# fabriziosestito/policy-server

Hardware: AMD Instinct MI355X
Metric: admission requests evaluated/sec (node) at 64 policies; HBM GB/s vs peak (higher is better)
Workload: dtype u8; 1 GPU; C4: 1000000 synthetic Pod AdmissionReviews per GPU x 64 compiled policies (c4_64.yml: 22 psp-capabilities, 21 psp-apparmor, 21 safe-labels); config=c4_64, total_requests=1000000, policies=64, parallelism=dp1 (request shards)

## Files before the change

### include/kwgpu.h

```cpp
#ifndef KWGPU_H
#define KWGPU_H

#include <stddef.h>
#include <stdint.h>

#ifdef __cplusplus
extern "C" {
#endif

enum {
  KW_OK = 0,
  KW_E_INVALID_ID = 1,
  KW_E_INIT = 2,
  KW_E_NOT_FOUND = 3,
  KW_E_BOOTSTRAP = 4,
  KW_E_ENGINE = 5,
  KW_E_GROUP_REHYDRATE = 6,
  KW_E_ARG = 16,
  KW_E_PAYLOAD = 17,
  KW_E_DEVICE = 18,
  KW_E_NOSPACE = 19
};

enum { KW_MODE_PROTECT = 0, KW_MODE_MONITOR = 1 };
// ... 117 lines not shown
int kw_batch_to_device(kw_batch *b, int device);
int kw_batch_to_device_async(kw_batch *b, int device, void *stream);
int kw_stream_create(int device, void **stream);
void kw_stream_destroy(void *stream);
void kw_batch_destroy(kw_batch *b);

int kw_debug_host_walk(const kw_env *env, const kw_batch *b, const int32_t *policies, uint32_t npol,
                       int origin, uint32_t *out);

int kw_debug_plan(const kw_env *env, kw_batch *b, const int32_t *policies, uint32_t npol, int origin, uint32_t *out,
                  int cap);

int kw_debug_copy_jobs(const kw_env *env, kw_batch *b, const int32_t *policies, uint32_t npol, int origin,
                       uint32_t *out, size_t cap, size_t *needed);

int kw_debug_reorder(const kw_batch *b, uint64_t *perm, size_t cap, uint64_t *split, kw_batch **out);

int kw_validate_batch(const kw_env *env, kw_batch *b, const int32_t *policies, uint32_t npol,
                      int origin, void *stream);
int kw_validate_rows(const kw_env *env, kw_batch *b, const int32_t *row_policy, int origin,
                     void *stream);
int kw_batch_verdicts(kw_batch *b, uint32_t *host_out, size_t count);
int kw_validate_host(const kw_env *env, kw_batch *b, const int32_t *policies, uint32_t npol, int origin,
                     int device, uint32_t *out, size_t count, uint32_t chunk_rows);
int kw_batch_pin_host(kw_batch *b, int device);
int kw_host_alloc(int device, size_t bytes, void **out);
void kw_host_free(void *p);
int kw_batch_wide_arg(const kw_batch *b, uint64_t row, int32_t policy, uint64_t *value);
int kw_batch_group_causes(const kw_batch *b, uint64_t row, int32_t policy, uint32_t verdict, uint64_t *words,
                          size_t nwords, size_t *needed);
// ... 41 lines not shown
```

### policy-server_amd/csrc/bulk.cpp

```cpp
#include <algorithm>
#include <chrono>
#include <cstdio>
#include <cstring>
#include <optional>

#include "bulkplan.hpp"
#include "knobs.hpp"
#include "pass.hpp"
#include "plan.hpp"
#include "upload.hpp"

namespace kw {
namespace {

using clk = std::chrono::steady_clock;
double since(clk::time_point a) { return std::chrono::duration<double, std::milli>(clk::now() - a).count(); }

struct BulkTimes {
  double layout = 0, plan = 0, prep = 0, desc = 0, fill = 0, enq = 0, out = 0, first = -1, wait = 0;
};

constexpr uint64_t kRing = 4;

struct Res {
// ... 228 lines not shown
        HIPCHK(hipMemcpyAsync(dslot, hslot, pk, hipMemcpyHostToDevice, s_in));
        HIPCHK(launch_scatter(sa, s_in));
      }
    } else {
      for (const CopySeg& c : segs)
        HIPCHK(hipMemcpyAsync(D.cols + ((uint8_t*)c.dst - st), c.dst, c.bytes, hipMemcpyHostToDevice, s_in));
    }
    t.enq += since(t1);
    return KW_OK;
  }

  int stage_descs(uint64_t k) {
    const auto td = clk::now();
    cd.clear();
    co.assign(1, 0u);
    if (int rc = build_descs(kb->b, pl.geom, 0, kb->b.n, tb[k], tb[k + 1], 128, &cd, &co)) return rc;
    co[0] = (uint32_t)(co.size() - 1);
    if (cd.size() > dcap) {
      HIPCHK(hipStreamSynchronize(res->s_in.s));
      HIPCHK(hipStreamSynchronize(sc));
      dcap = cd.size() + cd.size() / 4 + 64;
      if (int rc = alloc_descs()) return rc;
    } else if (k >= 2) {
      HIPCHK(hipEventSynchronize(res->ev[3 * (k - 2)]));
    }
    if (!cd.empty()) memcpy((TileDesc*)res->hdesc.p + (k & 1) * dcap, cd.data(), cd.size() * sizeof(TileDesc));
    t.desc += since(td);
    return KW_OK;
  }

  int launch(uint64_t k) {
// ... 115 lines not shown
```

### policy-server_amd/csrc/capi.cpp

```cpp
#include <hip/hip_runtime.h>

#include <algorithm>
#include <cstdio>
#include <cstdlib>
#include <cstring>
#include <memory>
#include <string>
#include <thread>
#include <vector>

#include "../../include/kwgpu.h"
#include "automaton.hpp"
#include "batch.hpp"
#include "devbatch.hpp"
#include "env.hpp"
#include "kernels.hpp"
#include "knobs.hpp"
#include "metrics.hpp"
#include "pass.hpp"
#include "plan.hpp"
#include "service.hpp"
#include "slotplan.hpp"
#include "upload.hpp"
#include "yaml.hpp"
// ... 539 lines not shown
  kb->dev = host_view(kb);
  const DeviceBatch& D = *kb->dev;
  const Batch& B = dev_rows(kb);
  PassPlan plan;
  int rc = plan_pass(env, kb, policies, npol, nullptr, origin, false, &plan);
  std::vector<uint32_t> w;
  if (rc == KW_OK) {
    const void* cols[kMaxCopyJobs] = {D.req_flags, D.ctr_off, D.lbl_off, D.ctr_flags, D.capadd_off, D.capdrop_off};
    for (int m = 0; m < (int)NSTR; ++m) cols[6 + 2 * m] = D.str[m].off, cols[7 + 2 * m] = D.str[m].bytes;
    w.push_back((uint32_t)plan.regions.size());
    for (const PassPlan::Region& rg : plan.regions) {
      const TileArgs& T = rg.geom;
      std::vector<TileDesc> desc;
      std::vector<uint32_t> ovf;
      const uint64_t ntiles = (rg.hi - rg.lo + T.rows - 1) / T.rows;
      if ((rc = build_descs(B, T, rg.lo, rg.hi, 0, ntiles, 4096, &desc, &ovf))) break;
      for (uint32_t v : {T.rows, T.njobs, (uint32_t)desc.size(), (uint32_t)ovf.size(), (uint32_t)rg.lo, (uint32_t)rg.hi, T.lds_bytes,
                         (uint32_t)D.split})
        w.push_back(v);
      for (uint32_t v : {T.o_rf, T.o_coff, T.o_loff, T.o_cflags, T.o_cadd, T.o_cdrop}) w.push_back(v);
      w.insert(w.end(), T.o_so, T.o_so + NSTR);
      w.insert(w.end(), T.o_sb, T.o_sb + NSTR);
      for (uint32_t j = 0; j < T.njobs; ++j) {
        const CopyJob& q = T.jobs[j];
        uint32_t col = 0xffffffffu;
        for (uint32_t c = 0; c < kMaxCopyJobs; ++c)
          if ((c < 6 || T.o_sb[(c - 6) / 2]) && q.base == (uint64_t)(uintptr_t)cols[c] && col == 0xffffffffu) col = c;
        for (uint32_t v : {col, copy_lds(q.code), (q.code & kCjX4) ? 16u : 4u, q.code}) w.push_back(v);
      }
      for (const TileDesc& d : desc) {
        const uint32_t* dw = (const uint32_t*)&d;
// ... 4 lines not shown
          for (uint32_t v : {(uint32_t)sp.byte_off, (uint32_t)(sp.byte_off >> 32), sp.count}) w.push_back(v);
        }
      }
      w.insert(w.end(), ovf.begin(), ovf.end());
    }
  }
  kb->dev->verdicts = nullptr;
  kb->dev = std::move(saved);
  if (rc) return rc;
  *needed = w.size();
  if (cap < w.size()) return KW_E_NOSPACE;
  std::copy(w.begin(), w.end(), out);
  return KW_OK;
}

int kw_debug_reorder(const kw_batch* kb, uint64_t* perm, size_t cap, uint64_t* split, kw_batch** out) {
  if (!kb || !split || !out || (!perm && kb->b.n) || cap < kb->b.n) return KW_E_ARG;
  std::vector<uint64_t> p;
  *split = split_rows(kb->b, &p);
  if (!*split) {
    p.resize(kb->b.n);
    for (uint64_t r = 0; r < kb->b.n; ++r) p[r] = r;
  }
  auto nb = std::make_unique<kw_batch>();
  RowOrder o;
  permute_batch(kb->b, p, &nb->b, true, &o);
  std::copy(p.begin(), p.end(), perm);
  *out = nb.release();
  return KW_OK;
}
// ... 136 lines not shown
```

### policy-server_amd/csrc/kernels.hip

```cpp
#include <hip/hip_runtime.h>

#include <algorithm>
#include <array>
#include <cstddef>
#include <mutex>

#include "../../include/kwgpu.h"
#include "imgscan.hpp"
#include "kernels.hpp"


namespace kw {

typedef uint32_t u32x4 __attribute__((ext_vector_type(4)));

__device__ inline uint32_t lit_word(const uint32_t* base, uint32_t i, uint32_t sh, uint32_t len) {
  const uint32_t w = align_bytes(base[i + 1], base[i], sh);
  const uint32_t rem = len - 4u * i;
  return rem >= 4u ? w : (w & ((1u << (8u * rem)) - 1u));
}

template <bool BATCH, int N = 8>
__device__ inline uint32_t lit_lookup(const uint8_t* rec, const uint8_t* bytes, uint32_t b, uint32_t e) {
  const DevLit* L = (const DevLit*)rec;
// ... 1123 lines not shown
      if (ck + 1 < t.nchunk) {
        if (DYNB && tid == 0) l_nx[3] = 0;
        lds_barrier();
        mark(4);
      }
    }
    const uint64_t p3_end = timing ? clock64() : 0;
    lds_barrier();
    if (timing) sg_add(SG_P3_WAIT, clock64() - p3_end);
    mark(4);
    tile = next;
    next = dyn ? dbase + l_nx[cur] : next + wpx;
  }
  if (timing && tid == 0) {
    ph[6] = clock64() - t_begin;
    for (int k = 0; k < 8; ++k) a.phase[(uint64_t)blockIdx.x * kPhaseWords + (uint32_t)k] = ph[k];
  }
  if (dyn && tid == 0) {
    uint32_t* done = a.sched + 256u + xcd * 32u;
    __threadfence();
    if (atomicAdd(done, 1u) == wpx - 1u) {
      atomicExch(cnt, 0u);
      atomicExch(done, 0u);
    }
  }
  (void)lane;
  (void)wave;
}

constexpr int kOverflowThreads = 256;
// ... 410 lines not shown
```

### policy-server_amd/csrc/kernels.hpp

```cpp
#pragma once
#include <hip/hip_runtime.h>

#include <cstdint>

#include "kwdev.hpp"
#include "slots.hpp"

namespace kw {

enum Str : uint32_t { S_NS = 0, S_IMG, S_AA, S_CAPADD, S_CAPDROP, S_LK, S_LV, NSTR };

struct WideRec {
  uint32_t row_lo, row_hi, policy, value;
};

struct EvalArgs {
  const uint8_t* blob;
  uint64_t nrows;
  uint64_t ndesc;
  uint32_t npol;
  int32_t origin;
  const uint8_t* req_flags;
  const uint32_t* ctr_off;
  const uint32_t* lbl_off;
// ... 5 lines not shown
  uint16_t *g_ns, *g_aa, *g_img, *g_capadd, *g_capdrop, *g_lk, *g_lv;
  const uint16_t *nfa_lv, *nfa_img;
  uint32_t* wide_count;
  WideRec* wide_rec;
  uint32_t wide_cap;
  uint64_t* wide_groups;
  uint32_t nwide;
  const uint32_t* rowcol;
  uint64_t* phase;
};
enum Seg : uint32_t {
  SG_P1_LABEL = 0, SG_P1_CAPSTR, SG_P1_CTR, SG_P1_IMAGE, SG_P1_REQ, SG_P2_CTR, SG_P2_LABEL, SG_P2_REQ,
  SG_P1_BUSY, SG_P1_WAIT, SG_P2_BUSY, SG_P2_WAIT, SG_P0_WAIT, SG_P3_BUSY, SG_P3_WAIT,
  SG_START,
  SG_P0_TOP, SG_P0_REQ, SG_P0_STR,
  kSegWords = 19
};
constexpr uint32_t kPhaseWords = 8 + kSegWords;

constexpr uint32_t kSlotRows = 64;
#ifndef KW_THREADS
#define KW_THREADS 256
#endif
constexpr uint32_t kSlotThreads = KW_THREADS;
constexpr uint32_t kLdsGranule = 1280, kLdsGranules = 128;
constexpr uint32_t lds_workgroups_per_cu(uint32_t bytes) {
  const uint32_t g = (bytes + kLdsGranule - 1) / kLdsGranule;
  return g ? kLdsGranules / g : kLdsGranules;
}
constexpr uint32_t kFeatImg = 1, kFeatLbl = 2, kFeatCtr = 4, kFeatGrp = 8, kFeatAll = 15;
constexpr uint32_t kFeatNfa = 16;
constexpr uint32_t kFeatRng = 32;
#ifndef KW_PREFETCH
// ... 75 lines not shown
  uint32_t debug;
  uint32_t lds_bytes;
};

struct alignas(16) TileDesc {
  uint32_t cb, ce, lb, le, kab, kae, kdb, kde;
  uint32_t sa[NSTR];
  uint32_t pad0;
  uint32_t nv[NSTR];
  uint32_t fits;
  uint32_t r0lo, r0hi, nr;
  uint32_t pad[4];
};
static_assert(sizeof(TileDesc) == 128, "TileDesc layout");

void build_copy_jobs(TileArgs* T, const void* const cols[6]);

hipError_t launch_evaluate_tiles(const EvalArgs& a, const TileArgs& t, const TileArgs* d_t, const TileDesc* d_desc,
                                 uint32_t grid, hipStream_t s);
struct WideGroupArgs {
  uint32_t prog_off, prog_len;
  uint32_t col;
  uint32_t nmem, midx_off;
  uint32_t okw, rejb;
  uint32_t cause_off, cause_words;
  uint32_t errw;
  uint32_t kind;
  uint32_t mutw;
};

// ... 64 lines not shown
```

### policy-server_amd/csrc/knobs.hpp

```cpp
#pragma once
#include <climits>
#include <cstddef>
#include <cstdint>

namespace kw {

enum Knob : int {
  KW_STREAM_POOL, KW_HOST_THREADS, KW_L2_PREFETCH, KW_KV_GLOBAL, KW_NO_MPACK,
  KW_BULK_DEBUG, KW_BULK_SAMPLE, KW_BULK_PACK, KW_BULK_CHUNK, KW_BULK_RAMP, KW_BULK_DIRECT, KW_BULK_DEPTH,
  KW_SCHED, KW_SPLIT, KW_GROUP_FORM, KW_POISON_VERDICTS, KW_FLATTEN_THREADS,
  KW_SLOT_ROWS, KW_HEAVY_ROWS, KW_HEAVY_CTR, KW_GLOBAL_TABLES, KW_TILE_SPLIT, KW_ROUND_SPLIT,
  KW_TILE_QUANTILE, KW_TILE_DEBUG,
  KW_NKNOBS
};

enum class KnobKind : uint8_t {
  On,
  Off,
  Present,
  Int,
  Double,
  Str
};

struct KnobRow {
  const char* name;
  KnobKind kind;
// ... 31 lines not shown
    knob_flag("KW_BULK_DIRECT", KnobKind::On, kLatched, kNoPlan, "bulk path: read back straight into pinned output"),
    knob_int("KW_BULK_DEPTH", kLatched, kNoPlan, -1, 0, INT_MAX, kClamp, "bulk path: chunks in flight (0: unbounded; unset: 2 or 3)"),
    knob_flag("KW_SCHED", KnobKind::Str, kLive, kPlans, "static / dynamic: force one tile schedule"),
    knob_int("KW_SPLIT", kLive, kPlans, -1, INT_MIN, INT_MAX, kClamp, "0: never split light / heavy rows, 1: whenever both exist"),
    knob_flag("KW_GROUP_FORM", KnobKind::Str, kLive, kPlans, "script: compile every group expression as a script"),
    knob_flag("KW_POISON_VERDICTS", KnobKind::Off, kLive, kPlans, "fill the verdict words with a sentinel before a pass"),
    knob_int("KW_FLATTEN_THREADS", kLive, kNoPlan, 0, 1, INT_MAX, kClamp, "JSON flatten threads (unset: the hardware's, at most 16)"),
    knob_int("KW_SLOT_ROWS", kLive, kPlans, 0, 8, 255, kElseUnset, "force the tile height"),
    knob_int("KW_HEAVY_ROWS", kLive, kPlans, 0, 8, 255, kElseUnset, "force the heavy region's tile height"),
    knob_int("KW_HEAVY_CTR", kLive, kPlans, 5, 1, INT_MAX, kElseUnset, "containers above which a request is heavy"),
    knob_flag("KW_GLOBAL_TABLES", KnobKind::Off, kLive, kPlans, "classifier tables read from global memory"),
    knob_real("KW_TILE_SPLIT", kPlans, 0.02, "share of tiles a capacity choice may split"),
    knob_real("KW_ROUND_SPLIT", kPlans, 0.02, "share of a taller tile's tiles that may need a second P1 round"),
    knob_real("KW_TILE_QUANTILE", kPlans, 0.0, "force the capacity quantile (unset: chosen per batch)"),
    knob_int("KW_TILE_DEBUG", kLive, kPlans, 0, INT_MIN, INT_MAX, kClamp, "kernel phase ablation bits; 256: print the plan"),
};

constexpr bool knob_name_is(const char* a, const char* b) {
  while (*a && *a == *b) ++a, ++b;
  return *a == *b;
}
#define KW_KNOB_ROW(K) static_assert(knob_name_is(kKnobs[K].name, #K), "kKnobs is not in Knob order")
KW_KNOB_ROW(KW_STREAM_POOL); KW_KNOB_ROW(KW_HOST_THREADS); KW_KNOB_ROW(KW_L2_PREFETCH); KW_KNOB_ROW(KW_KV_GLOBAL);
KW_KNOB_ROW(KW_NO_MPACK); KW_KNOB_ROW(KW_BULK_DEBUG); KW_KNOB_ROW(KW_BULK_SAMPLE); KW_KNOB_ROW(KW_BULK_PACK);
KW_KNOB_ROW(KW_BULK_CHUNK); KW_KNOB_ROW(KW_BULK_RAMP); KW_KNOB_ROW(KW_BULK_DIRECT); KW_KNOB_ROW(KW_BULK_DEPTH);
KW_KNOB_ROW(KW_SCHED); KW_KNOB_ROW(KW_SPLIT); KW_KNOB_ROW(KW_GROUP_FORM); KW_KNOB_ROW(KW_POISON_VERDICTS);
KW_KNOB_ROW(KW_FLATTEN_THREADS); KW_KNOB_ROW(KW_SLOT_ROWS); KW_KNOB_ROW(KW_HEAVY_ROWS); KW_KNOB_ROW(KW_HEAVY_CTR);
KW_KNOB_ROW(KW_GLOBAL_TABLES); KW_KNOB_ROW(KW_TILE_SPLIT); KW_KNOB_ROW(KW_ROUND_SPLIT); KW_KNOB_ROW(KW_TILE_QUANTILE);
KW_KNOB_ROW(KW_TILE_DEBUG);
#undef KW_KNOB_ROW

uint64_t kw_knob_hash();

namespace knob_detail {

const char* env(const KnobRow& r);
bool parse_bool(const KnobRow& r);
int parse_int(const KnobRow& r);
double parse_double(const KnobRow& r);

template <Knob K>
bool latched_bool() {
  static const bool v = parse_bool(kKnobs[K]);
  return v;
// ... 57 lines not shown
```

### policy-server_amd/csrc/pass.cpp

```cpp
#include "pass.hpp"

#include <atomic>
#include <chrono>
#include <cstdio>
#include <cstring>
#include <memory>

#include "knobs.hpp"
#include "plan.hpp"

namespace kw {

int upload_env(kw_env* env, int device) {
  if (device < 0) return KW_OK;
  HIPCHK(hipSetDevice(device));
  HIPCHK(hipMalloc(&env->e.d_blob, env->e.blob.size()));
  HIPCHK(hipMemcpy(env->e.d_blob, env->e.blob.data(), env->e.blob.size(), hipMemcpyHostToDevice));
  env->e.device = device;
  return KW_OK;
}

int build_descs(const Batch& B, const TileArgs& T, uint64_t lo, uint64_t hi, uint64_t t0, uint64_t t1, uint64_t range,
                std::vector<TileDesc>* desc, std::vector<uint32_t>* ovf) {
  auto make = [&](uint64_t r0, uint64_t r1, TileDesc* dp) {
    TileDesc& d = *dp;
    memset(&d, 0, sizeof(d));
    d.r0lo = (uint32_t)r0;
    d.r0hi = (uint32_t)(r0 >> 32);
    d.nr = (uint32_t)(r1 - r0);
    d.cb = B.ctr_off[r0];
    d.ce = B.ctr_off[r1];
    d.lb = B.lbl_off[r0];
    d.le = B.lbl_off[r1];
    d.kab = B.capadd_off[d.cb];
    d.kae = B.capadd_off[d.ce];
    d.kdb = B.capdrop_off[d.cb];
    d.kde = B.capdrop_off[d.ce];
    bool fits = d.ce - d.cb <= T.cmax && d.kae - d.kab <= T.kmax && d.kde - d.kdb <= T.kmax && d.le - d.lb <= T.lmax;
    for (int m = 0; m < (int)NSTR; ++m) {
      if (!T.o_sb[m]) continue;
      uint64_t g0, g1;
      str_range(B, m, r0, r1, &g0, &g1);
      const StrCol& c = host_str(B, m);
      d.sa[m] = c.off[g0] & ~15u;
      d.nv[m] = (((c.off[g1] + 15u) & ~15u) - d.sa[m]) / 16u;
      fits = fits && d.nv[m] * 16u <= T.sb_cap[m];
    }
    d.fits = fits ? 1u : 0u;
    return fits;
  };
  const size_t nq = (size_t)((t1 - t0 + range - 1) / range);
  std::vector<std::vector<TileDesc>> qdesc(nq);
  std::vector<std::vector<uint32_t>> qovf(nq);
  std::atomic<bool> too_far{false};
  HostWorkers::get().run(nq, [&](size_t q) {
    std::vector<std::pair<uint64_t, uint64_t>> todo;
    std::vector<TileDesc>& dv = qdesc[q];
    dv.reserve((size_t)range + range / 64);
    for (uint64_t tile = t0 + q * range, te = std::min<uint64_t>(t1, t0 + (q + 1) * range); tile < te; ++tile) {
      todo.assign(1, {lo + tile * T.rows, std::min<uint64_t>(hi, lo + (tile + 1) * T.rows)});
      while (!todo.empty()) {
        const auto [r0, r1] = todo.back();
        todo.pop_back();
        TileDesc d;
        if (make(r0, r1, &d)) {
          dv.push_back(d);
        } else if (r1 - r0 > 1) {
          const uint64_t mid = r0 + (r1 - r0) / 2;
          todo.push_back({mid, r1});
          todo.push_back({r0, mid});
        } else {
          if (r0 > 0xffffffffull) too_far = true;
          qovf[q].push_back((uint32_t)r0);
        }
      }
    }
  });
  if (too_far) return KW_E_ARG;
  for (size_t q = 0; q < nq; ++q) {
    desc->insert(desc->end(), qdesc[q].begin(), qdesc[q].end());
    ovf->insert(ovf->end(), qovf[q].begin(), qovf[q].end());
  }
  return KW_OK;
}

static int upload_tile_descs(const Batch& B, DeviceBatch* D, const PassPlan& plan, hipStream_t s) {
  uint64_t key = 1469598103934665603ull;
  auto mix = [&](uint64_t v) { key = (key ^ v) * 1099511628211ull; };
  for (const PassPlan::Region& rg : plan.regions) {
    const TileArgs& T = rg.geom;
    mix(rg.lo);
    mix(rg.hi);
    mix(T.rows);
    mix(T.cmax);
    mix(T.kmax);
    mix(T.lmax);
    for (int m = 0; m < (int)NSTR; ++m) {
      mix(T.o_sb[m] != 0);
      mix(T.sb_cap[m]);
    }
  }
  if (D->desc && D->desc_valid && key == D->desc_key) return KW_OK;
  const bool dbg = Knobs::on<KW_BULK_DEBUG>();
  const auto t0 = std::chrono::steady_clock::now();
  std::vector<TileDesc> desc;
  std::vector<uint32_t> ovf{0};
  if (plan.regions.size() > 2) return KW_E_ARG;
  uint64_t at[2] = {0, 0}, nd[2] = {0, 0};
  for (size_t k = 0; k < plan.regions.size(); ++k) {
    const PassPlan::Region& rg = plan.regions[k];
    const uint64_t ntiles = (rg.hi - rg.lo + rg.geom.rows - 1) / rg.geom.rows;
    at[k] = desc.size();
    desc.reserve(desc.size() + ntiles + ntiles / 64 + 1);
    if (int rc = build_descs(B, rg.geom, rg.lo, rg.hi, 0, ntiles, 4096, &desc, &ovf)) return rc;
    nd[k] = desc.size() - at[k];
  }
  ovf[0] = (uint32_t)(ovf.size() - 1);
  const auto t1 = std::chrono::steady_clock::now();
  HIPCHK(hipStreamSynchronize(s));
  D->h_desc = std::move(desc);
  D->h_ovf = std::move(ovf);
  if (int rc = ensure(&D->desc, &D->desc_cap, std::max<size_t>(D->h_desc.size(), 1))) return rc;
  if (int rc = ensure(&D->overflow, &D->overflow_cap, D->h_ovf.size())) return rc;
  if (!D->h_desc.empty())
    HIPCHK(hipMemcpyAsync(D->desc, D->h_desc.data(), D->h_desc.size() * sizeof(TileDesc), hipMemcpyHostToDevice, s));
  D->ndesc = D->h_desc.size();
  for (int k = 0; k < 2; ++k) {
    D->reg_desc[k] = at[k];
    D->reg_ndesc[k] = nd[k];
  }
  HIPCHK(hipMemcpyAsync(D->overflow, D->h_ovf.data(), D->h_ovf.size() * sizeof(uint32_t), hipMemcpyHostToDevice, s));
  D->n_overflow = D->h_ovf[0];
// ... 164 lines not shown
          g[SG_P1_CTR] / wt, g[SG_P1_IMAGE] / wt, g[SG_P1_REQ] / wt, g[SG_P2_BUSY] / wt, g[SG_P2_WAIT] / wt,
          g[SG_P2_CTR] / wt, g[SG_P2_LABEL] / wt, g[SG_P2_REQ] / wt, g[SG_P3_BUSY] / wt, g[SG_P3_WAIT] / wt,
          g[SG_P0_TOP] / wt, g[SG_P0_REQ] / wt, g[SG_P0_STR] / wt);
  const uint32_t nx = std::min(8u, grid);
  uint32_t late = 0;
  double spread = 0;
  for (uint32_t x = 0; x < nx; ++x) {
    std::vector<uint64_t> st;
    for (uint32_t q = x; q < grid; q += nx) st.push_back(ph[(size_t)q * kPhaseWords + 8 + SG_START]);
    std::sort(st.begin(), st.end());
    for (uint64_t v : st) late += v > st[0] + 2000;
    spread = std::max(spread, (double)(st.back() - st[0]) / 100.0);
  }
  fprintf(stderr, "[kw start] launch %zu: %u of %u workgroups started > 20 us after their XCD's first (widest spread %.1f us)\n",
          launch, late, grid, spread);
}

static int run_pass(kw_batch* kb, PassPlan& plan, bool timed, hipStream_t s) {
  DeviceBatch& D = *kb->dev;
  EvalArgs A;
  if (int rc = prepare_pass(kb, plan, s, &A)) return rc;
  const bool phases = (plan.geom.debug & 512u) != 0;
  void* d_phase = nullptr;
  uint32_t gmax = 0;
  for (const PassPlan::Region& rg : plan.regions) gmax = std::max(gmax, rg.grid);
  const size_t phase_bytes = (size_t)gmax * kPhaseWords * sizeof(uint64_t);
  if (phases) {
    HIPCHK(hipMalloc(&d_phase, phase_bytes));
    A.phase = (uint64_t*)d_phase;
  }
// ... 264 lines not shown
```

### policy-server_amd/csrc/pass.hpp

```cpp
#pragma once
#include <hip/hip_runtime.h>

#include <algorithm>
#include <cstdint>
#include <vector>

#include "devbatch.hpp"

#define HIPCHK(x)                             \
  do {                                        \
    hipError_t _e = (x);                      \
    if (_e != hipSuccess) return KW_E_DEVICE; \
  } while (0)

namespace kw {

template <typename T>
int ensure(T** p, size_t* cap, size_t n) {
  if (*cap >= n && *p) return KW_OK;
  int dev = 0;
  HIPCHK(hipGetDevice(&dev));
  dev_pool().release(dev, *p, *cap * sizeof(T));
  *p = nullptr;
  const size_t want = BlockPool::cls(std::max<size_t>(n, 1) * sizeof(T)) / sizeof(T);
  void* q = nullptr;
  HIPCHK(dev_pool().alloc(dev, want * sizeof(T), &q));
  *p = (T*)q;
  *cap = want;
  return KW_OK;
}

int upload_env(kw_env* env, int device);

int build_descs(const Batch& B, const TileArgs& T, uint64_t lo, uint64_t hi, uint64_t t0, uint64_t t1, uint64_t range,
                std::vector<TileDesc>* desc, std::vector<uint32_t>* ovf);

int ensure_overflow_classes(const Batch& B, DeviceBatch* D, const TileArgs& T, EvalArgs* A);

int prepare_pass(kw_batch* kb, PassPlan& plan, hipStream_t s, EvalArgs* out_args, bool descs = true);

int run_validate(const kw_env* env, kw_batch* kb, PassPlan& plan, int origin, bool timed, hipStream_t s);

int validate_common(const kw_env* env, kw_batch* kb, const int32_t* policies, uint32_t npol, const int32_t* row_policy,
                    int origin, PassPlan* plan);

int validate_cached(const kw_env* env, kw_batch* kb, const int32_t* policies, uint32_t npol, int origin, PassPlan** out);

int validate_timed(const kw_env* env, kw_batch* b, const int32_t* policies, uint32_t npol, int origin, int warmup, int reps,
                   kw_timing* out);

// ... 6 lines not shown
```

### policy-server_amd/kwgpu/__init__.py

```python
import ctypes as C
import json

from . import _native as N
from ._native import KwSoa, KwTiming

PROTECT, MONITOR = N.KW_MODE_PROTECT, N.KW_MODE_MONITOR
VALIDATE, AUDIT = N.KW_ORIGIN_VALIDATE, N.KW_ORIGIN_AUDIT


class RequestOrigin:
    Validate = N.KW_ORIGIN_VALIDATE
    Audit = N.KW_ORIGIN_AUDIT


class PolicyMode:
    Protect = N.KW_MODE_PROTECT
    Monitor = N.KW_MODE_MONITOR


class EvaluationError(Exception):

    code = None

    def __init__(self, message, code=None):
# ... 345 lines not shown
        keys = ("lds_bytes", "launches", "chunks", "lds_tables", "rows", "cmax", "kmax", "lmax", "regions", "split",
                "grid", "heavy_lds_bytes", "heavy_rows", "heavy_cmax", "heavy_grid", "scan_regions")
        return dict(zip(keys, out[:16]))

    def debug_copy_jobs(self, env, policies, origin=VALIDATE):
        import numpy as np
        arr = env._array(policies)
        need = C.c_size_t()
        rc = self._L.kw_debug_copy_jobs(env._h, self._h, arr, len(policies), origin, None, 0, C.byref(need))
        if rc != N.KW_E_NOSPACE:
            raise_for(rc, "kw_debug_copy_jobs failed")
        out = np.zeros(max(need.value, 1), dtype=np.uint32)
        rc = self._L.kw_debug_copy_jobs(env._h, self._h, arr, len(policies), origin,
                                        out.ctypes.data_as(C.POINTER(C.c_uint32)), out.size, C.byref(need))
        raise_for(rc, "kw_debug_copy_jobs failed")
        return out[:need.value]

    def debug_reorder(self):
        import numpy as np
        perm = np.zeros(max(self.n, 1), dtype=np.uint64)
        split, h = C.c_uint64(), C.c_void_p()
        rc = self._L.kw_debug_reorder(self._h, perm.ctypes.data_as(C.POINTER(C.c_uint64)), len(perm), C.byref(split),
                                      C.byref(h))
        raise_for(rc, "kw_debug_reorder failed")
        return Batch(h.value), perm[:self.n], split.value

    def wide_arg(self, row, policy):
        v = C.c_uint64()
        rc = self._L.kw_batch_wide_arg(self._h, row, policy, C.byref(v))
        return v.value if rc == N.KW_OK else None
# ... 206 lines not shown
```

### policy-server_amd/kwgpu/_native.py

```python
import ctypes as C
import os

PKG_DIR = os.path.dirname(os.path.dirname(os.path.abspath(__file__)))
LIB_PATH = os.environ.get("KWGPU_LIB") or os.path.join(PKG_DIR, "libkwgpu.so")
SYNTH_PATH = os.path.join(PKG_DIR, "libkwsynth.so")

KW_OK = 0
KW_E_INVALID_ID = 1
KW_E_INIT = 2
KW_E_NOT_FOUND = 3
KW_E_BOOTSTRAP = 4
KW_E_ENGINE = 5
KW_E_GROUP_REHYDRATE = 6
KW_E_ARG = 16
KW_E_PAYLOAD = 17
KW_E_DEVICE = 18
KW_E_NOSPACE = 19

KW_MODE_PROTECT = 0
KW_MODE_MONITOR = 1
KW_ORIGIN_VALIDATE = 0
KW_ORIGIN_AUDIT = 1
KW_DOC_ADMISSION_REVIEW = 0
KW_DOC_RAW_REVIEW = 1
# ... 40 lines not shown
    _fields_ = [("continue_on_errors", C.c_int), ("always_accept_namespace", C.c_char_p), ("device", C.c_int)]


class KwTiming(C.Structure):
    _fields_ = [("classify_ms", C.c_double), ("evaluate_ms", C.c_double), ("total_ms", C.c_double),
                ("classify_bytes", C.c_double), ("evaluate_bytes", C.c_double)]


EXPORTS = [
    "kw_env_build", "kw_env_build_yaml", "kw_yaml_to_json", "kw_env_serialize", "kw_env_deserialize", "kw_env_destroy", "kw_env_lookup",
    "kw_env_policy_count", "kw_env_policy_id", "kw_env_is_group", "kw_env_get_policy_mode",
    "kw_env_get_policy_allowed_to_mutate",
    "kw_env_should_always_accept_requests_made_inside_of_namespace",
    "kw_env_policy_initialization_error", "kw_env_validate_settings", "kw_pattern_match", "kw_pattern_match_many", "kw_env_pattern_count",
    "kw_env_pattern", "kw_env_classify", "kw_batch_wide_arg", "kw_batch_group_causes", "kw_debug_plan", "kw_debug_copy_jobs", "kw_debug_reorder",
    "kw_batch_from_json", "kw_batch_from_soa", "kw_batch_view", "kw_batch_to_device", "kw_batch_to_device_async",
    "kw_stream_create", "kw_stream_destroy", "kw_validate_host", "kw_batch_pin_host", "kw_host_alloc", "kw_host_free",
    "kw_batch_destroy", "kw_debug_host_walk", "kw_validate_batch", "kw_validate_rows", "kw_batch_verdicts",
    "kw_validate_timed", "kw_format_response", "kw_format_response_doc", "kw_env_group_members", "kw_evaluate",
    "kw_service_constraints", "kw_metrics_create", "kw_metrics_destroy", "kw_metrics_record", "kw_metrics_render",
    "kw_metrics_reset", "kw_version",
]

_lib = None
_synth = None


def lib():
    global _lib
    if _lib is not None:
# ... 20 lines not shown
        "kw_env_is_group": (ip, [vp, i32]),
        "kw_env_get_policy_mode": (ip, [vp, i32, C.POINTER(ip)]),
        "kw_env_get_policy_allowed_to_mutate": (ip, [vp, i32, C.POINTER(ip)]),
        "kw_env_should_always_accept_requests_made_inside_of_namespace": (ip, [vp, cp, sz]),
        "kw_env_policy_initialization_error": (ip, [vp, i32, cp, sz]),
        "kw_env_validate_settings": (ip, [vp, i32, cp, sz]),
        "kw_pattern_match": (ip, [ip, cp, cp, sz]),
        "kw_pattern_match_many": (ip, [ip, cp, C.POINTER(cp), C.POINTER(sz), sz, C.POINTER(C.c_int32)]),
        "kw_env_pattern_count": (ip, [vp, ip]),
        "kw_env_pattern": (ip, [vp, ip, ip, C.POINTER(ip), cp, sz]),
        "kw_env_classify": (ip, [vp, ip, cp, sz, cp, sz, C.POINTER(u32), ip]),
        "kw_batch_wide_arg": (ip, [vp, u64, i32, C.POINTER(u64)]),
        "kw_batch_group_causes": (ip, [vp, u64, i32, C.c_uint32, C.POINTER(u64), C.c_size_t, C.POINTER(C.c_size_t)]),
        "kw_debug_plan": (ip, [vp, vp, C.POINTER(i32), u32, ip, C.POINTER(u32), ip]),
        "kw_debug_copy_jobs": (ip, [vp, vp, C.POINTER(i32), u32, ip, C.POINTER(u32), sz, C.POINTER(sz)]),
        "kw_debug_reorder": (ip, [vp, C.POINTER(u64), sz, C.POINTER(u64), C.POINTER(vp)]),
        "kw_batch_from_json": (ip, [C.POINTER(cp), C.POINTER(sz), sz, ip, C.POINTER(vp), C.POINTER(C.c_int64), cp, sz]),
        "kw_batch_from_soa": (ip, [C.POINTER(KwSoa), C.POINTER(vp)]),
        "kw_batch_view": (ip, [vp, C.POINTER(KwSoa)]),
        "kw_batch_to_device": (ip, [vp, ip]),
        "kw_batch_to_device_async": (ip, [vp, ip, vp]),
        "kw_stream_create": (ip, [ip, C.POINTER(vp)]),
        "kw_stream_destroy": (None, [vp]),
        "kw_batch_destroy": (None, [vp]),
        "kw_validate_batch": (ip, [vp, vp, C.POINTER(i32), u32, ip, vp]),
        "kw_validate_rows": (ip, [vp, vp, C.POINTER(i32), ip, vp]),
        "kw_batch_verdicts": (ip, [vp, C.POINTER(u32), sz]),
        "kw_validate_host": (ip, [vp, vp, C.POINTER(i32), u32, ip, ip, C.POINTER(u32), sz, u32]),
        "kw_batch_pin_host": (ip, [vp, ip]),
        "kw_host_alloc": (ip, [ip, sz, C.POINTER(vp)]),
# ... 45 lines not shown
```

Baseline: 4.157 billion requests/s.

## Cut tiles at the row with least estimated cost per row

Adds a cost model (fixed plus per-64-item block weights for requests, labels, containers and capabilities) and, behind a knob that is on by default, lets each tile end up to an eighth of its height early, at the row that minimises estimated cost per row. Each 4096-tile range keeps the cut version only if its total estimated cost drops, and cutting is dropped everywhere if it would raise the most per-XCD rounds under the tile-to-XCD slot mapping. The aim is to even out work per tile and cut wasted padding work. The cost is more host-side planning work and more descriptors. Also adds end-of-workgroup timestamps, per-XCD idle reporting and debug APIs.

```diff
diff --git a/include/kwgpu.h b/include/kwgpu.h
--- a/include/kwgpu.h
+++ b/include/kwgpu.h
@@ -155,6 +155,14 @@
 int kw_debug_copy_jobs(const kw_env *env, kw_batch *b, const int32_t *policies, uint32_t npol, int origin,
                        uint32_t *out, size_t cap, size_t *needed);
 
+int kw_debug_tile_descs(const kw_env *env, kw_batch *b, const int32_t *policies, uint32_t npol, int origin,
+                        uint32_t *out, size_t cap, size_t *needed);
+
+uint64_t kw_debug_tile_cost(uint32_t feat, uint32_t need, uint32_t requests, uint32_t labels, uint32_t containers,
+                            uint32_t capabilities);
+
+int kw_debug_tile_slot(uint64_t ndesc, uint32_t grid, uint32_t workgroup, uint32_t tile, uint64_t *out);
+
 int kw_debug_reorder(const kw_batch *b, uint64_t *perm, size_t cap, uint64_t *split, kw_batch **out);
 
 int kw_validate_batch(const kw_env *env, kw_batch *b, const int32_t *policies, uint32_t npol,
diff --git a/policy-server_amd/csrc/bulk.cpp b/policy-server_amd/csrc/bulk.cpp
--- a/policy-server_amd/csrc/bulk.cpp
+++ b/policy-server_amd/csrc/bulk.cpp
@@ -266,7 +266,7 @@
     const auto td = clk::now();
     cd.clear();
     co.assign(1, 0u);
-    if (int rc = build_descs(kb->b, pl.geom, 0, kb->b.n, tb[k], tb[k + 1], 128, &cd, &co)) return rc;
+    if (int rc = build_descs(kb->b, pl.geom, 0, kb->b.n, tb[k], tb[k + 1], 128, 0, &cd, &co)) return rc;
     co[0] = (uint32_t)(co.size() - 1);
     if (cd.size() > dcap) {
       HIPCHK(hipStreamSynchronize(res->s_in.s));
diff --git a/policy-server_amd/csrc/capi.cpp b/policy-server_amd/csrc/capi.cpp
--- a/policy-server_amd/csrc/capi.cpp
+++ b/policy-server_amd/csrc/capi.cpp
@@ -577,7 +577,7 @@
       std::vector<TileDesc> desc;
       std::vector<uint32_t> ovf;
       const uint64_t ntiles = (rg.hi - rg.lo + T.rows - 1) / T.rows;
-      if ((rc = build_descs(B, T, rg.lo, rg.hi, 0, ntiles, 4096, &desc, &ovf))) break;
+      if ((rc = build_descs(B, T, rg.lo, rg.hi, 0, ntiles, 4096, rg.grid, &desc, &ovf))) break;
       for (uint32_t v : {T.rows, T.njobs, (uint32_t)desc.size(), (uint32_t)ovf.size(), (uint32_t)rg.lo, (uint32_t)rg.hi, T.lds_bytes,
                          (uint32_t)D.split})
         w.push_back(v);
@@ -612,6 +612,65 @@
   return KW_OK;
 }
 
+int kw_debug_tile_descs(const kw_env* env, kw_batch* kb, const int32_t* policies, uint32_t npol, int origin, uint32_t* out,
+                        size_t cap, size_t* needed) {
+  if (!env || !kb || !needed || (!out && cap) || (!policies && npol)) return KW_E_ARG;
+  std::unique_ptr<DeviceBatch> saved = std::move(kb->dev);
+  kb->dev = host_view(kb);
+  const Batch& B = dev_rows(kb);
+  PassPlan plan;
+  int rc = plan_pass(env, kb, policies, npol, nullptr, origin, false, &plan);
+  std::vector<uint32_t> w;
+  if (rc == KW_OK) {
+    std::vector<TileDesc> desc;
+    std::vector<uint32_t> ovf;
+    uint64_t at[2] = {0, 0}, nd[2] = {0, 0};
+    rc = plan_descs(B, plan, &desc, &ovf, at, nd);
+    if (rc == KW_OK) {
+      w.push_back((uint32_t)plan.regions.size());
+      w.push_back(ovf[0]);
+      for (size_t k = 0; k < plan.regions.size(); ++k) {
+        const PassPlan::Region& rg = plan.regions[k];
+        const TileArgs& T = rg.geom;
+        const TileCostW W = tile_cost_weights(T.feat, T.need);
+        for (uint32_t v : {T.rows, T.cmax, T.kmax, T.lmax, rg.grid, tile_slot(nd[k], rg.grid, 0).nx, rg.dyn ? 1u : 0u,
+                           (uint32_t)nd[k], (uint32_t)rg.lo, (uint32_t)rg.hi})
+          w.push_back(v);
+        for (int m = 0; m < (int)NSTR; ++m) w.push_back(T.o_sb[m] ? 1u : 0u);
+        w.insert(w.end(), T.sb_cap, T.sb_cap + NSTR);
+        for (uint64_t i = at[k]; i < at[k] + nd[k]; ++i) {
+          const uint32_t* dw = (const uint32_t*)&desc[i];
+          w.insert(w.end(), dw, dw + sizeof(TileDesc) / 4);
+          const uint64_t c = desc_cost(W, desc[i]);
+          w.push_back((uint32_t)c);
+          w.push_back((uint32_t)(c >> 32));
+        }
+      }
+      w.insert(w.end(), ovf.begin() + 1, ovf.end());
+    }
+  }
+  kb->dev->verdicts = nullptr;
+  kb->dev = std::move(saved);
+  if (rc) return rc;
+  *needed = w.size();
+  if (cap < w.size()) return KW_E_NOSPACE;
+  std::copy(w.begin(), w.end(), out);
+  return KW_OK;
+}
+
+uint64_t kw_debug_tile_cost(uint32_t feat, uint32_t need, uint32_t requests, uint32_t labels, uint32_t containers,
+                            uint32_t capabilities) {
+  return tile_cost(tile_cost_weights(feat, need), requests, labels, containers, capabilities);
+}
+
+int kw_debug_tile_slot(uint64_t ndesc, uint32_t grid, uint32_t workgroup, uint32_t tile, uint64_t* out) {
+  if (!out || !grid || workgroup >= grid) return KW_E_ARG;
+  const TileSlot s = tile_slot(ndesc, grid, workgroup);
+  const uint64_t v[7] = {s.nx, s.xcd, s.slot, s.wpx, s.t_lo, s.t_hi, tile_at(s, tile)};
+  std::copy(v, v + 7, out);
+  return KW_OK;
+}
+
 int kw_debug_reorder(const kw_batch* kb, uint64_t* perm, size_t cap, uint64_t* split, kw_batch** out) {
   if (!kb || !split || !out || (!perm && kb->b.n) || cap < kb->b.n) return KW_E_ARG;
   std::vector<uint64_t> p;
diff --git a/policy-server_amd/csrc/kernels.hip b/policy-server_amd/csrc/kernels.hip
--- a/policy-server_amd/csrc/kernels.hip
+++ b/policy-server_amd/csrc/kernels.hip
@@ -1161,6 +1161,7 @@
   }
   if (timing && tid == 0) {
     ph[6] = clock64() - t_begin;
+    a.phase[(uint64_t)blockIdx.x * kPhaseWords + 8u + SG_END] = __builtin_amdgcn_s_memrealtime();
     for (int k = 0; k < 8; ++k) a.phase[(uint64_t)blockIdx.x * kPhaseWords + (uint32_t)k] = ph[k];
   }
   if (dyn && tid == 0) {
diff --git a/policy-server_amd/csrc/kernels.hpp b/policy-server_amd/csrc/kernels.hpp
--- a/policy-server_amd/csrc/kernels.hpp
+++ b/policy-server_amd/csrc/kernels.hpp
@@ -43,9 +43,11 @@
   SG_P1_BUSY, SG_P1_WAIT, SG_P2_BUSY, SG_P2_WAIT, SG_P0_WAIT, SG_P3_BUSY, SG_P3_WAIT,
   SG_START,
   SG_P0_TOP, SG_P0_REQ, SG_P0_STR,
-  kSegWords = 19
-};
-constexpr uint32_t kPhaseWords = 8 + kSegWords;
+  SG_END,
+  kSegWords = 20
+};
+constexpr uint32_t kPhaseWords = 32;
+static_assert(kPhaseWords >= 8 + kSegWords && kPhaseWords % 16 == 0, "phase words per workgroup: whole lines");
 
 constexpr uint32_t kSlotRows = 64;
 #ifndef KW_THREADS
@@ -151,6 +153,39 @@
 };
 static_assert(sizeof(TileDesc) == 128, "TileDesc layout");
 
+struct TileSlot {
+  uint32_t nx, xcd, slot, wpx;
+  uint64_t t_lo, t_hi;
+};
+KW_HD inline TileSlot tile_slot(uint64_t ndesc, uint32_t grid, uint32_t b) {
+  TileSlot s;
+  s.nx = grid < 8u ? grid : 8u;
+  s.xcd = b % s.nx;
+  s.slot = b / s.nx;
+  s.wpx = (grid - s.xcd + s.nx - 1u) / s.nx;
+  s.t_lo = ndesc * s.xcd / s.nx;
+  s.t_hi = ndesc * (s.xcd + 1u) / s.nx;
+  return s;
+}
+KW_HD inline uint64_t tile_at(const TileSlot& s, uint32_t k) { return s.t_lo + s.slot + (uint64_t)k * s.wpx; }
+
+struct TileCostW {
+  uint32_t fixed, req, lbl, ctr, cap;
+};
+KW_HD constexpr uint32_t tile_blocks(uint32_t items) { return (items + 63u) / 64u; }
+KW_HD constexpr uint64_t tile_cost(const TileCostW& w, uint32_t nreq, uint32_t nlbl, uint32_t nctr, uint32_t ncap) {
+  return (uint64_t)w.fixed + (uint64_t)w.req * tile_blocks(nreq) + (uint64_t)w.lbl * tile_blocks(nlbl) +
+         (uint64_t)w.ctr * tile_blocks(nctr) + (uint64_t)w.cap * tile_blocks(ncap);
+}
+KW_HD constexpr TileCostW tile_cost_weights(uint32_t feat, uint32_t need) {
+  TileCostW w{47000u, 8450u, 0u, 0u, 0u};
+  if ((feat & kFeatLbl) && (need & (1u << S_LK))) w.lbl = 9960u;
+  if (feat & kFeatCtr) w.ctr = 10600u;
+  if ((feat & kFeatCtr) && (need & (1u << S_CAPADD))) w.cap = 2750u;
+  if ((feat & kFeatImg) && (need & (1u << S_IMG))) w.ctr = 35600u;
+  return w;
+}
+
 void build_copy_jobs(TileArgs* T, const void* const cols[6]);
 
 hipError_t launch_evaluate_tiles(const EvalArgs& a, const TileArgs& t, const TileArgs* d_t, const TileDesc* d_desc,
diff --git a/policy-server_amd/csrc/knobs.hpp b/policy-server_amd/csrc/knobs.hpp
--- a/policy-server_amd/csrc/knobs.hpp
+++ b/policy-server_amd/csrc/knobs.hpp
@@ -10,7 +10,7 @@
   KW_BULK_DEBUG, KW_BULK_SAMPLE, KW_BULK_PACK, KW_BULK_CHUNK, KW_BULK_RAMP, KW_BULK_DIRECT, KW_BULK_DEPTH,
   KW_SCHED, KW_SPLIT, KW_GROUP_FORM, KW_POISON_VERDICTS, KW_FLATTEN_THREADS,
   KW_SLOT_ROWS, KW_HEAVY_ROWS, KW_HEAVY_CTR, KW_GLOBAL_TABLES, KW_TILE_SPLIT, KW_ROUND_SPLIT,
-  KW_TILE_QUANTILE, KW_TILE_DEBUG,
+  KW_TILE_QUANTILE, KW_TILE_DEBUG, KW_TILE_CUT,
   KW_NKNOBS
 };
 
@@ -72,6 +72,7 @@
     knob_real("KW_ROUND_SPLIT", kPlans, 0.02, "share of a taller tile's tiles that may need a second P1 round"),
     knob_real("KW_TILE_QUANTILE", kPlans, 0.0, "force the capacity quantile (unset: chosen per batch)"),
     knob_int("KW_TILE_DEBUG", kLive, kPlans, 0, INT_MIN, INT_MAX, kClamp, "kernel phase ablation bits; 256: print the plan"),
+    knob_flag("KW_TILE_CUT", KnobKind::On, kLive, kPlans, "end each tile at the row of least estimated cost per row (0: fixed height)"),
 };
 
 constexpr bool knob_name_is(const char* a, const char* b) {
@@ -85,7 +86,7 @@
 KW_KNOB_ROW(KW_SCHED); KW_KNOB_ROW(KW_SPLIT); KW_KNOB_ROW(KW_GROUP_FORM); KW_KNOB_ROW(KW_POISON_VERDICTS);
 KW_KNOB_ROW(KW_FLATTEN_THREADS); KW_KNOB_ROW(KW_SLOT_ROWS); KW_KNOB_ROW(KW_HEAVY_ROWS); KW_KNOB_ROW(KW_HEAVY_CTR);
 KW_KNOB_ROW(KW_GLOBAL_TABLES); KW_KNOB_ROW(KW_TILE_SPLIT); KW_KNOB_ROW(KW_ROUND_SPLIT); KW_KNOB_ROW(KW_TILE_QUANTILE);
-KW_KNOB_ROW(KW_TILE_DEBUG);
+KW_KNOB_ROW(KW_TILE_DEBUG); KW_KNOB_ROW(KW_TILE_CUT);
 #undef KW_KNOB_ROW
 
 uint64_t kw_knob_hash();
diff --git a/policy-server_amd/csrc/pass.cpp b/policy-server_amd/csrc/pass.cpp
--- a/policy-server_amd/csrc/pass.cpp
+++ b/policy-server_amd/csrc/pass.cpp
@@ -21,7 +21,7 @@
 }
 
 int build_descs(const Batch& B, const TileArgs& T, uint64_t lo, uint64_t hi, uint64_t t0, uint64_t t1, uint64_t range,
-                std::vector<TileDesc>* desc, std::vector<uint32_t>* ovf) {
+                uint32_t grid, std::vector<TileDesc>* desc, std::vector<uint32_t>* ovf) {
   auto make = [&](uint64_t r0, uint64_t r1, TileDesc* dp) {
     TileDesc& d = *dp;
     memset(&d, 0, sizeof(d));
@@ -49,48 +49,110 @@
     d.fits = fits ? 1u : 0u;
     return fits;
   };
+  const bool cut = Knobs::on<KW_TILE_CUT>() && grid && (T.feat & (kFeatLbl | kFeatCtr));
+  const TileCostW W = tile_cost_weights(T.feat, T.need);
+  auto cost = [&](uint64_t r0, uint64_t r1) {
+    const uint32_t cb = B.ctr_off[r0], ce = B.ctr_off[r1];
+    return tile_cost(W, (uint32_t)(r1 - r0), B.lbl_off[r1] - B.lbl_off[r0], ce - cb,
+                     (B.capadd_off[ce] - B.capadd_off[cb]) + (B.capdrop_off[ce] - B.capdrop_off[cb]));
+  };
   const size_t nq = (size_t)((t1 - t0 + range - 1) / range);
-  std::vector<std::vector<TileDesc>> qdesc(nq);
-  std::vector<std::vector<uint32_t>> qovf(nq);
+  std::vector<std::vector<TileDesc>> qdesc[2] = {std::vector<std::vector<TileDesc>>(nq), std::vector<std::vector<TileDesc>>(nq)};
+  std::vector<std::vector<uint32_t>> qovf[2] = {std::vector<std::vector<uint32_t>>(nq), std::vector<std::vector<uint32_t>>(nq)};
+  std::vector<uint8_t> qcut(nq, 0);
   std::atomic<bool> too_far{false};
   HostWorkers::get().run(nq, [&](size_t q) {
     std::vector<std::pair<uint64_t, uint64_t>> todo;
-    std::vector<TileDesc>& dv = qdesc[q];
-    dv.reserve((size_t)range + range / 64);
-    for (uint64_t tile = t0 + q * range, te = std::min<uint64_t>(t1, t0 + (q + 1) * range); tile < te; ++tile) {
-      todo.assign(1, {lo + tile * T.rows, std::min<uint64_t>(hi, lo + (tile + 1) * T.rows)});
-      while (!todo.empty()) {
-        const auto [r0, r1] = todo.back();
-        todo.pop_back();
-        TileDesc d;
-        if (make(r0, r1, &d)) {
-          dv.push_back(d);
-        } else if (r1 - r0 > 1) {
-          const uint64_t mid = r0 + (r1 - r0) / 2;
-          todo.push_back({mid, r1});
-          todo.push_back({r0, mid});
-        } else {
-          if (r0 > 0xffffffffull) too_far = true;
-          qovf[q].push_back((uint32_t)r0);
+    const uint64_t qb = lo + (t0 + q * range) * T.rows;
+    const uint64_t qe = std::min<uint64_t>(hi, lo + std::min<uint64_t>(t1, t0 + (q + 1) * range) * T.rows);
+    uint64_t total[2] = {0, 0};
+    for (int v = 0; v <= (cut ? 1 : 0); ++v) {
+      std::vector<TileDesc>& dv = qdesc[v][q];
+      dv.reserve((size_t)range + (v ? range / 8 : 0) + range / 64 + 1);
+      for (uint64_t r = std::min(qb, qe); r < qe;) {
+        uint64_t end = std::min<uint64_t>(qe, r + T.rows);
+        if (v && end < qe) {
+          uint64_t best = cost(r, end);
+          for (uint64_t e = end - 1; e >= r + T.rows - T.rows / 8 && e > r; --e) {
+            const uint64_t c = cost(r, e);
+            if (c * (end - r) < best * (e - r)) best = c, end = e;
+          }
+        }
+        todo.assign(1, {r, end});
+        r = end;
+        while (!todo.empty()) {
+          const auto [r0, r1] = todo.back();
+          todo.pop_back();
+          TileDesc d;
+          if (make(r0, r1, &d)) {
+            dv.push_back(d);
+            total[v] += desc_cost(W, d);
+          } else if (r1 - r0 > 1) {
+            const uint64_t mid = r0 + (r1 - r0) / 2;
+            todo.push_back({mid, r1});
+            todo.push_back({r0, mid});
+          } else {
+            if (r0 > 0xffffffffull) too_far = true;
+            qovf[v][q].push_back((uint32_t)r0);
+          }
         }
       }
     }
+    qcut[q] = cut && total[1] < total[0];
   });
   if (too_far) return KW_E_ARG;
+  if (cut) {
+    uint64_t n[2] = {0, 0};
+    for (size_t q = 0; q < nq; ++q) n[0] += qdesc[0][q].size(), n[1] += qdesc[qcut[q]][q].size();
+    auto rounds = [&](uint64_t nd) {
+      uint64_t most = 0;
+      for (uint32_t x = 0; x < tile_slot(nd, grid, 0).nx; ++x) {
+        const TileSlot ts = tile_slot(nd, grid, x);
+        most = std::max(most, (ts.t_hi - ts.t_lo + ts.wpx - 1) / ts.wpx);
+      }
+      return most;
+    };
+    if (rounds(n[1]) > rounds(n[0])) std::fill(qcut.begin(), qcut.end(), 0);
+  }
   for (size_t q = 0; q < nq; ++q) {
-    desc->insert(desc->end(), qdesc[q].begin(), qdesc[q].end());
-    ovf->insert(ovf->end(), qovf[q].begin(), qovf[q].end());
-  }
+    desc->insert(desc->end(), qdesc[qcut[q]][q].begin(), qdesc[qcut[q]][q].end());
+    ovf->insert(ovf->end(), qovf[qcut[q]][q].begin(), qovf[qcut[q]][q].end());
+  }
+  return KW_OK;
+}
+
+uint64_t desc_cost(const TileCostW& w, const TileDesc& d) {
+  return d.fits ? tile_cost(w, d.nr, d.le - d.lb, d.ce - d.cb, (d.kae - d.kab) + (d.kde - d.kdb)) : 0;
+}
+
+int plan_descs(const Batch& B, const PassPlan& plan, std::vector<TileDesc>* desc, std::vector<uint32_t>* ovf, uint64_t at[2],
+               uint64_t nd[2]) {
+  desc->clear();
+  ovf->assign(1, 0u);
+  if (plan.regions.size() > 2) return KW_E_ARG;
+  for (size_t k = 0; k < plan.regions.size(); ++k) {
+    const PassPlan::Region& rg = plan.regions[k];
+    const uint64_t ntiles = (rg.hi - rg.lo + rg.geom.rows - 1) / rg.geom.rows;
+    at[k] = desc->size();
+    desc->reserve(desc->size() + ntiles + ntiles / 8 + ntiles / 64 + 1);
+    if (int rc = build_descs(B, rg.geom, rg.lo, rg.hi, 0, ntiles, 4096, rg.grid, desc, ovf)) return rc;
+    nd[k] = desc->size() - at[k];
+  }
+  (*ovf)[0] = (uint32_t)(ovf->size() - 1);
   return KW_OK;
 }
 
 static int upload_tile_descs(const Batch& B, DeviceBatch* D, const PassPlan& plan, hipStream_t s) {
   uint64_t key = 1469598103934665603ull;
   auto mix = [&](uint64_t v) { key = (key ^ v) * 1099511628211ull; };
+  mix(Knobs::on<KW_TILE_CUT>());
   for (const PassPlan::Region& rg : plan.regions) {
     const TileArgs& T = rg.geom;
     mix(rg.lo);
     mix(rg.hi);
+    mix(rg.grid);
+    mix(T.feat);
+    mix(T.need);
     mix(T.rows);
     mix(T.cmax);
     mix(T.kmax);
@@ -104,18 +166,9 @@
   const bool dbg = Knobs::on<KW_BULK_DEBUG>();
   const auto t0 = std::chrono::steady_clock::now();
   std::vector<TileDesc> desc;
-  std::vector<uint32_t> ovf{0};
-  if (plan.regions.size() > 2) return KW_E_ARG;
+  std::vector<uint32_t> ovf;
   uint64_t at[2] = {0, 0}, nd[2] = {0, 0};
-  for (size_t k = 0; k < plan.regions.size(); ++k) {
-    const PassPlan::Region& rg = plan.regions[k];
-    const uint64_t ntiles = (rg.hi - rg.lo + rg.geom.rows - 1) / rg.geom.rows;
-    at[k] = desc.size();
-    desc.reserve(desc.size() + ntiles + ntiles / 64 + 1);
-    if (int rc = build_descs(B, rg.geom, rg.lo, rg.hi, 0, ntiles, 4096, &desc, &ovf)) return rc;
-    nd[k] = desc.size() - at[k];
-  }
-  ovf[0] = (uint32_t)(ovf.size() - 1);
+  if (int rc = plan_descs(B, plan, &desc, &ovf, at, nd)) return rc;
   const auto t1 = std::chrono::steady_clock::now();
   HIPCHK(hipStreamSynchronize(s));
   D->h_desc = std::move(desc);
@@ -310,6 +363,28 @@
   }
   fprintf(stderr, "[kw start] launch %zu: %u of %u workgroups started > 20 us after their XCD's first (widest spread %.1f us)\n",
           launch, late, grid, spread);
+  fprintf(stderr, "[kw finish] launch %zu: per XCD end spread us / idle share:", launch);
+  double idle_all = 0, span_all = 0;
+  uint32_t stamped = 0;
+  for (uint32_t x = 0; x < nx; ++x) {
+    uint64_t first = ~0ull, e_lo = ~0ull, e_hi = 0, n = 0, ends = 0;
+    for (uint32_t q = x; q < grid; q += nx) {
+      const uint64_t* w = &ph[(size_t)q * kPhaseWords + 8];
+      if (!w[SG_START] || !w[SG_END]) continue;
+      ++n;
+      first = std::min(first, w[SG_START]);
+      e_lo = std::min(e_lo, w[SG_END]);
+      e_hi = std::max(e_hi, w[SG_END]);
+      ends += w[SG_END];
+    }
+    const double idle = (double)n * (double)e_hi - (double)ends, span = (double)n * (double)(e_hi - first);
+    idle_all += idle;
+    span_all += span;
+    stamped += (uint32_t)n;
+    fprintf(stderr, " %.1f / %.1f %%", (double)(e_hi - e_lo) / 100.0, span > 0 ? 100.0 * idle / span : 0.0);
+  }
+  fprintf(stderr, " (all: %.1f %% idle; %u of %u workgroups stamped)\n", span_all > 0 ? 100.0 * idle_all / span_all : 0.0,
+          stamped, grid);
 }
 
 static int run_pass(kw_batch* kb, PassPlan& plan, bool timed, hipStream_t s) {
diff --git a/policy-server_amd/csrc/pass.hpp b/policy-server_amd/csrc/pass.hpp
--- a/policy-server_amd/csrc/pass.hpp
+++ b/policy-server_amd/csrc/pass.hpp
@@ -33,7 +33,12 @@
 int upload_env(kw_env* env, int device);
 
 int build_descs(const Batch& B, const TileArgs& T, uint64_t lo, uint64_t hi, uint64_t t0, uint64_t t1, uint64_t range,
-                std::vector<TileDesc>* desc, std::vector<uint32_t>* ovf);
+                uint32_t grid, std::vector<TileDesc>* desc, std::vector<uint32_t>* ovf);
+
+uint64_t desc_cost(const TileCostW& w, const TileDesc& d);
+
+int plan_descs(const Batch& B, const PassPlan& plan, std::vector<TileDesc>* desc, std::vector<uint32_t>* ovf, uint64_t at[2],
+               uint64_t nd[2]);
 
 int ensure_overflow_classes(const Batch& B, DeviceBatch* D, const TileArgs& T, EvalArgs* A);
 
diff --git a/policy-server_amd/kwgpu/__init__.py b/policy-server_amd/kwgpu/__init__.py
--- a/policy-server_amd/kwgpu/__init__.py
+++ b/policy-server_amd/kwgpu/__init__.py
@@ -383,6 +383,19 @@
         rc = self._L.kw_debug_copy_jobs(env._h, self._h, arr, len(policies), origin,
                                         out.ctypes.data_as(C.POINTER(C.c_uint32)), out.size, C.byref(need))
         raise_for(rc, "kw_debug_copy_jobs failed")
+        return out[:need.value]
+
+    def debug_tile_descs(self, env, policies, origin=VALIDATE):
+        import numpy as np
+        arr = env._array(policies)
+        need = C.c_size_t()
+        rc = self._L.kw_debug_tile_descs(env._h, self._h, arr, len(policies), origin, None, 0, C.byref(need))
+        if rc != N.KW_E_NOSPACE:
+            raise_for(rc, "kw_debug_tile_descs failed")
+        out = np.zeros(max(need.value, 1), dtype=np.uint32)
+        rc = self._L.kw_debug_tile_descs(env._h, self._h, arr, len(policies), origin,
+                                         out.ctypes.data_as(C.POINTER(C.c_uint32)), out.size, C.byref(need))
+        raise_for(rc, "kw_debug_tile_descs failed")
         return out[:need.value]
 
     def debug_reorder(self):
diff --git a/policy-server_amd/kwgpu/_native.py b/policy-server_amd/kwgpu/_native.py
--- a/policy-server_amd/kwgpu/_native.py
+++ b/policy-server_amd/kwgpu/_native.py
@@ -78,6 +78,7 @@
     "kw_env_should_always_accept_requests_made_inside_of_namespace",
     "kw_env_policy_initialization_error", "kw_env_validate_settings", "kw_pattern_match", "kw_pattern_match_many", "kw_env_pattern_count",
     "kw_env_pattern", "kw_env_classify", "kw_batch_wide_arg", "kw_batch_group_causes", "kw_debug_plan", "kw_debug_copy_jobs", "kw_debug_reorder",
+    "kw_debug_tile_descs", "kw_debug_tile_cost", "kw_debug_tile_slot",
     "kw_batch_from_json", "kw_batch_from_soa", "kw_batch_view", "kw_batch_to_device", "kw_batch_to_device_async",
     "kw_stream_create", "kw_stream_destroy", "kw_validate_host", "kw_batch_pin_host", "kw_host_alloc", "kw_host_free",
     "kw_batch_destroy", "kw_debug_host_walk", "kw_validate_batch", "kw_validate_rows", "kw_batch_verdicts",
@@ -128,6 +129,9 @@
         "kw_batch_group_causes": (ip, [vp, u64, i32, C.c_uint32, C.POINTER(u64), C.c_size_t, C.POINTER(C.c_size_t)]),
         "kw_debug_plan": (ip, [vp, vp, C.POINTER(i32), u32, ip, C.POINTER(u32), ip]),
         "kw_debug_copy_jobs": (ip, [vp, vp, C.POINTER(i32), u32, ip, C.POINTER(u32), sz, C.POINTER(sz)]),
+        "kw_debug_tile_descs": (ip, [vp, vp, C.POINTER(i32), u32, ip, C.POINTER(u32), sz, C.POINTER(sz)]),
+        "kw_debug_tile_cost": (u64, [u32, u32, u32, u32, u32, u32]),
+        "kw_debug_tile_slot": (ip, [u64, u32, u32, u32, C.POINTER(u64)]),
         "kw_debug_reorder": (ip, [vp, C.POINTER(u64), sz, C.POINTER(u64), C.POINTER(vp)]),
         "kw_batch_from_json": (ip, [C.POINTER(cp), C.POINTER(sz), sz, ip, C.POINTER(vp), C.POINTER(C.c_int64), cp, sz]),
         "kw_batch_from_soa": (ip, [C.POINTER(KwSoa), C.POINTER(vp)]),
```

Result: faster. 4.305 billion requests/s, median of 6 (+3.6%).
